# hermosayhl/CNN

Measured on AMD Instinct MI355X. Metric: images/sec (train step, 224x224x3), higher is better.
Workload: dtype f32; 1 GPU; reference AlexNet-style net (cpu/src/alexnet.cpp:10-33: 4x Conv3x3/s2 + ReLU, one MaxPool2x2, Linear 4608->3), full train step (fwd + softmax/CE + bwd + SGD), 224x224x3 fp32, BASELINE configs[1]; per_gpu_batch=256, global_batch=256, parallelism=dp1

## Files before the change

### cnn_amd/csrc/conv_direct.hip

```cpp
#include <cstdlib>

#include "conv_families.h"

using namespace cnn_amd;

namespace {

constexpr int kWaves = 4;
constexpr int kBlock = 64 * kWaves;

template <int CI, int CO, int K, int S>
__global__ __launch_bounds__(kBlock) void conv_direct_fwd(const float* __restrict__ x, const float* __restrict__ w,
                                                          const float* __restrict__ bias, float* __restrict__ y,
                                                          float* __restrict__ y_relu, int B, int H, int W, int Ho,
                                                          int Wo) {
    const int lane = threadIdx.x & 63;
    const int wave = __builtin_amdgcn_readfirstlane(threadIdx.x >> 6);
    const long long rows = (long long)B * Ho;
    for (long long r = (long long)blockIdx.x * kWaves + wave; r < rows; r += (long long)gridDim.x * kWaves) {
        const int b = (int)(r / Ho), p = (int)(r - (long long)b * Ho);
        const float* xb = x + (size_t)b * CI * H * W + (size_t)(p * S) * W;
        float* yb = y + (size_t)b * CO * Ho * Wo + (size_t)p * Wo;
        float* rb = y_relu ? y_relu + (size_t)b * CO * Ho * Wo + (size_t)p * Wo : nullptr;
        for (int q = lane; q < Wo; q += 64) {
// ... 496 lines not shown
    pack_fwd_3_16_3_2_body(w, bias, wp, threadIdx.x, blockDim.x);
}

struct PackJob {
    int kind;
    const float* w;
    const float* bias;
    float* out;
    int CI, CO;
};
struct PackBatch {
    int n;
    PackJob j[8];
};
__global__ void pack_batch(const PackBatch pb) {
    const PackJob& jb = pb.j[blockIdx.y];
    const int tid = blockIdx.x * blockDim.x + threadIdx.x, nt = gridDim.x * blockDim.x;
    if (jb.kind == 0) pack_fwd_3_16_3_2_body(jb.w, jb.bias, jb.out, tid, nt);
    else if (jb.kind == 1) pack_dgrad_3_16_3_2_body(jb.w, jb.out, tid);
    else pack_dgrad_s2_body(jb.w, jb.out, jb.CI, jb.CO, tid, nt);
}

constexpr int kFinThreads = 1024, kFinLanes = 8, kFinN = 16 * 28;
__global__ __launch_bounds__(kFinThreads) void first_layer_finish(const float* __restrict__ slabs, int nslots, float divisor,
                                                                  float* __restrict__ gw, float* __restrict__ gb, float* __restrict__ w,
                                                                  float* __restrict__ bias, float lr, float scale, int scaled,
                                                                  float* __restrict__ fwd_img, float* __restrict__ dgrad_img,
                                                                  float* __restrict__ w_keep, float* __restrict__ bias_keep) {
    __shared__ float red[kFinLanes][kFinN];
    __shared__ float wl[16 * 27], bl[16];
    constexpr int PAIRS = kFinLanes * kFinN, PER = (PAIRS + kFinThreads - 1) / kFinThreads;
    float acc[PER];
    int idx[PER], sl[PER];
#pragma unroll
    for (int q = 0; q < PER; ++q) {
        const int pr = threadIdx.x + q * kFinThreads;
        acc[q] = 0.f;
        sl[q] = pr / kFinN;
        idx[q] = pr - sl[q] * kFinN;
    }
    const bool last_live = threadIdx.x + (PER - 1) * kFinThreads < PAIRS;
    if (!last_live) idx[PER - 1] = 0, sl[PER - 1] = 0;
    constexpr int kBatch = 8;
    for (int s0 = 0; s0 < nslots; s0 += kBatch * kFinLanes) {
        float v[kBatch][PER];
#pragma unroll
        for (int u = 0; u < kBatch; ++u)
#pragma unroll
            for (int q = 0; q < PER; ++q) {
                const int s = s0 + u * kFinLanes + sl[q];
                v[u][q] = slabs[(size_t)(s < nslots ? s : 0) * kFinN + idx[q]];
            }
#pragma unroll
        for (int u = 0; u < kBatch; ++u)
#pragma unroll
            for (int q = 0; q < PER; ++q) {
                const float sum = acc[q] + v[u][q];
                acc[q] = (s0 + u * kFinLanes + sl[q] < nslots) ? sum : acc[q];
            }
    }
#pragma unroll
    for (int q = 0; q < PER; ++q)
        if (q + 1 < PER || last_live) red[sl[q]][idx[q]] = acc[q];
    __syncthreads();
    if (threadIdx.x < kFinN) {
        const int i = threadIdx.x;
        float t = 0.f;
#pragma unroll
        for (int k = 0; k < kFinLanes; ++k) t += red[k][i];
        const float g = t / divisor;
        const int row = i / 28, col = i - row * 28;
        if (col < 27) {
            const int j = row * 27 + col;
            gw[j] = g;
            const float old = w[j];
            if (w_keep) w_keep[j] = old;
            const float v = sgd_one(old, g, lr, scale, scaled != 0);
            w[j] = v;
            wl[j] = v;
        } else {
            if (gb) gb[row] = g;
            const float oldb = bias ? bias[row] : 0.f;
            if (bias && bias_keep) bias_keep[row] = oldb;
            const float v = bias ? sgd_one(oldb, g, lr, scale, scaled != 0) : 0.f;
            if (bias) bias[row] = v;
            bl[row] = v;
        }
    }
    __syncthreads();
    if (fwd_img) pack_fwd_3_16_3_2_body(wl, bl, fwd_img, threadIdx.x, kFinThreads);
    if (dgrad_img) pack_dgrad_3_16_3_2_body(wl, dgrad_img, threadIdx.x);
}

constexpr int kDR = 4;
constexpr int kDSeg = 62;
template <int MODE>
__global__ __launch_bounds__(kBlock) void conv_dgrad_pool_lds_3_16_3_2(const float* __restrict__ dpool, const int32_t* __restrict__ pmask,
                                                                       const float* __restrict__ pooled, const v2f* __restrict__ wp,
                                                                       float* __restrict__ dx, int B, int H, int W, int Ho, int Wo,
                                                                       int ngroups, int nsegs, unsigned m_gs, unsigned m_seg) {
    constexpr bool RM = MODE == 1, PK8 = MODE == 2;
    constexpr int CO = 16, CI = 3, NA = RM ? 3 : 2, ROWS = kDR + 1;
    static_assert(kDR == kWaves, "one block row per wave");
    __shared__ float tile[NA][CO][ROWS][64];
    const int U = (H + 1) / 2, V = (W + 1) / 2, U2 = (U + 1) / 2, V2 = (V + 1) / 2;
    const int PHo = Ho / 2, PWo = Wo / 2, pplane = PHo * PWo, plane = Ho * Wo;
    const int lane = threadIdx.x & 63;
    const int wave = __builtin_amdgcn_readfirstlane(threadIdx.x >> 6);
    const int pbytes = (int)((unsigned)B * CO * pplane * 4u);
    const int pitch8 = pool_mask_pitch(PWo), plane8 = PHo * pitch8;
    const __amdgpu_buffer_rsrc_t rd = __builtin_amdgcn_make_buffer_rsrc((void*)dpool, 0, pbytes, 0x00020000);
    const __amdgpu_buffer_rsrc_t rm = __builtin_amdgcn_make_buffer_rsrc((void*)pmask, 0, PK8 ? (int)((unsigned)B * CO * plane8) : pbytes, 0x00020000);
    const __amdgpu_buffer_rsrc_t rp = __builtin_amdgcn_make_buffer_rsrc((void*)(RM ? pooled : dpool), 0, pbytes, 0x00020000);
    const int item = (int)xcd_swizzle(blockIdx.x, gridDim.x);
    const int gs = ngroups * nsegs;
    const int b = fast_div(item, m_gs, gs);
    const int rem = item - b * gs;
    const int grp = fast_div(rem, m_seg, nsegs), sg = rem - grp * nsegs;
    const int bh0 = grp * kDR, bw0 = sg * kDSeg;
    {
        const int wc = bw0 - 1 + lane;
        const bool cok = wc >= 0 && wc < PWo && lane <= kDSeg;
        constexpr int PER = CO * ROWS / kWaves;
        float vd[PER], vm[PER], vp[RM ? PER : 1];
#pragma unroll
        for (int jj = 0; jj < PER; ++jj) {
            const int j = jj * kWaves + wave;
            const int ch = j / ROWS, r = j - ch * ROWS;
            const int wr = bh0 - 1 + r;
            const unsigned off = (cok && wr >= 0 && wr < PHo) ? (unsigned)(wr * PWo + wc) * 4u : kBufOOB;
            const int so = (b * CO + ch) * pplane * 4;
            vd[jj] = __builtin_bit_cast(float, __builtin_amdgcn_raw_buffer_load_b32(rd, (int)off, so, 0));
            if constexpr (PK8) {
                const unsigned off8 = (off != kBufOOB) ? (unsigned)(wr * pitch8 + wc) : kBufOOB;
                vm[jj] = __builtin_bit_cast(float, (int)__builtin_amdgcn_raw_buffer_load_b8(rm, (int)off8, (b * CO + ch) * plane8, 0));
            } else
                vm[jj] = __builtin_bit_cast(float, __builtin_amdgcn_raw_buffer_load_b32(rm, (int)off, so, 0));
            if constexpr (RM) vp[jj] = __builtin_bit_cast(float, __builtin_amdgcn_raw_buffer_load_b32(rp, (int)off, so, 0));
        }
#pragma unroll
        for (int jj = 0; jj < PER; ++jj) {
            const int j = jj * kWaves + wave;
            const int ch = j / ROWS, r = j - ch * ROWS;
            tile[0][ch][r][lane] = vd[jj];
            tile[1][ch][r][lane] = vm[jj];
            if constexpr (RM) tile[2][ch][r][lane] = vp[jj];
        }
    }
    __syncthreads();
    const int bh = bh0 + wave, bw = bw0 + lane;
    if (bh >= U2) return;
    const bool live = lane < kDSeg && bw < V2;
    const int e00 = (2 * bh - 1) * Wo + (2 * bw - 1);
    v2f acc[4][6];
#pragma unroll
    for (int sb = 0; sb < 4; ++sb)
#pragma unroll
        for (int k = 0; k < 6; ++k) acc[sb][k] = v2f{0.f, 0.f};
    const int l1 = lane < 63 ? lane + 1 : 63;
#pragma unroll 2
    for (int ch = 0; ch < CO; ++ch) {
        float g[4], pl[4];
        int mk[4];
#pragma unroll
        for (int w = 0; w < 4; ++w) {
            const int r = wave + (w >> 1), sl = (w & 1) ? l1 : lane;
            g[w] = tile[0][ch][r][sl];
            mk[w] = __builtin_bit_cast(int, tile[1][ch][r][sl]);
            if constexpr (RM) pl[w] = tile[2][ch][r][sl];
            else pl[w] = 1.f;
        }
        float D[3][3];
        const int cbase = ch * plane + e00;
#pragma unroll
        for (int w = 0; w < 4; ++w) g[w] = (pl[w] <= 0.f) ? 0.f : g[w];
#pragma unroll
        for (int i = 0; i < 3; ++i)
#pragma unroll
            for (int j = 0; j < 3; ++j) {
                const int w = ((i + 1) >> 1) * 2 + ((j + 1) >> 1);
                if constexpr (PK8) D[i][j] = (mk[w] == ((i + 1) & 1) * 2 + ((j + 1) & 1)) ? g[w] : 0.f;
                else D[i][j] = (mk[w] == cbase + i * Wo + j) ? g[w] : 0.f;
            }
        asm volatile("" ::: "memory");
        const v2f* q = wp + ch * 16;
#pragma unroll
        for (int sb = 0; sb < 4; ++sb) {
            const int sr = sb >> 1, sc = sb & 1;
            const v2f a = {D[sr + 1][sc + 1], D[sr + 1][sc + 1]}, bq = {D[sr + 1][sc], D[sr + 1][sc]},
                      c = {D[sr][sc + 1], D[sr][sc + 1]}, e = {D[sr][sc], D[sr][sc]};
            v2f& P0 = acc[sb][0]; v2f& P1 = acc[sb][1]; v2f& P2 = acc[sb][2]; v2f& P3 = acc[sb][3];
            v2f& Q0 = acc[sb][4]; v2f& Q1 = acc[sb][5];
            P0 = __builtin_elementwise_fma(q[0], a, P0);
            P1 = __builtin_elementwise_fma(q[1], a, P1);
            P2 = __builtin_elementwise_fma(q[2], a, P2);
            P3 = __builtin_elementwise_fma(q[3], a, P3);
            Q0 = __builtin_elementwise_fma(q[4], a, Q0);
            Q1 = __builtin_elementwise_fma(q[5], a, Q1);
            P0 = __builtin_elementwise_fma(q[6], bq, P0);
            P2 = __builtin_elementwise_fma(q[7], bq, P2);
            Q0 = __builtin_elementwise_fma(q[8], bq, Q0);
            Q1 = __builtin_elementwise_fma(q[9], bq, Q1);
            P0 = __builtin_elementwise_fma(q[10], c, P0);
            P1 = __builtin_elementwise_fma(q[11], c, P1);
            Q0 = __builtin_elementwise_fma(q[12], c, Q0);
            P0 = __builtin_elementwise_fma(q[13], e, P0);
            Q0 = __builtin_elementwise_fma(q[14], e, Q0);
        }
    }
    if (!live) return;
    float* dxb = dx + (size_t)b * CI * H * W;
    const bool quad = (W & 3) == 0;
#pragma unroll
    for (int ci = 0; ci < CI; ++ci)
#pragma unroll
        for (int rr = 0; rr < 4; ++rr) {
            const int sr = rr >> 1, ph = rr & 1, h = 4 * bh + rr;
            float v[4];
#pragma unroll
            for (int sc = 0; sc < 2; ++sc) {
                const v2f* A = acc[sr * 2 + sc];
                if (ci == 2) {
                    v[2 * sc] = ph ? A[5].x : A[4].x;
                    v[2 * sc + 1] = ph ? A[5].y : A[4].y;
                } else {
                    const v2f lo = ph ? A[2] : A[0], hi = ph ? A[3] : A[1];
                    v[2 * sc] = ci ? lo.y : lo.x;
                    v[2 * sc + 1] = ci ? hi.y : hi.x;
                }
            }
            if (h >= H) continue;
            float* row = dxb + ((size_t)ci * H + h) * W + 4 * (size_t)bw;
            if (quad) {
                {
                    typedef float nt4 __attribute__((ext_vector_type(4)));
                    __builtin_nontemporal_store(nt4{v[0], v[1], v[2], v[3]}, (nt4*)row);
                }
            } else {
#pragma unroll
                for (int k = 0; k < 4; ++k)
                    if (4 * bw + k < W) row[k] = v[k];
            }
        }
}

typedef int v2i __attribute__((ext_vector_type(2)));

template <bool RELU>
__global__ __launch_bounds__(kBlock) void conv_fwd_pk_3_16_3_2(const float* __restrict__ x, const v2f* __restrict__ wp,
                                                               float* __restrict__ y, float* __restrict__ y_relu, int B,
                                                               int H, int W, int Ho, int Wo, int items_per_img,
                                                               unsigned m_ipi, unsigned m_row) {
    constexpr int CI = 3, CO = 16, K = 3;
    const int lane = threadIdx.x & 63;
    const int wave = __builtin_amdgcn_readfirstlane(threadIdx.x >> 6);
    const long long items = (long long)B * items_per_img;
    const int plane = Ho * Wo;
    for (int it = xcd_swizzle(blockIdx.x, gridDim.x) * kWaves + wave; it < (int)items; it += gridDim.x * kWaves) {
        const int b = fast_div(it, m_ipi, items_per_img);
        const int n = (it - b * items_per_img) * 64 + lane;
        const bool live = n < plane;
        const int p = fast_div(live ? n : 0, m_row, Wo), q = (live ? n : 0) - p * Wo;
        const unsigned vo = live ? (unsigned)(2 * p * W + 2 * q) : 0u;
        float patch[CI * K * K];
#pragma unroll
        for (int ci = 0; ci < CI; ++ci)
#pragma unroll
            for (int kx = 0; kx < K; ++kx) {
                const float* rowp = x + (size_t)((b * CI + ci) * H + kx) * W;
                const f3u pr = *(const f3u*)(rowp + vo);
                patch[(ci * K + kx) * K + 0] = pr.x;
                patch[(ci * K + kx) * K + 1] = pr.y;
                patch[(ci * K + kx) * K + 2] = pr.z;
            }
        v2f acc[CO / 2];
#pragma unroll
        for (int j = 0; j < CO / 2; ++j) acc[j] = v2f{0.f, 0.f};
#pragma unroll
        for (int t = 0; t < CI * K * K; ++t) {
            asm volatile("" ::: "memory");
            const v2f* qw = wp + t * (CO / 2);
            const v2f pv = {patch[t], patch[t]};
#pragma unroll
            for (int j = 0; j < CO / 2; ++j) acc[j] = __builtin_elementwise_fma(qw[j], pv, acc[j]);
        }
        if (!live) continue;
        const v2f* qb = wp + CI * K * K * (CO / 2);
        float* yb = y + (size_t)b * CO * plane + n;
        float* rb = RELU ? y_relu + (size_t)b * CO * plane + n : nullptr;
#pragma unroll
        for (int j = 0; j < CO / 2; ++j) {
            const v2f v = acc[j] + qb[j];
            yb[(size_t)(2 * j) * plane] = v.x;
            yb[(size_t)(2 * j + 1) * plane] = v.y;
            if (RELU) {
                rb[(size_t)(2 * j) * plane] = v.x >= 0.f ? v.x : 0.f;
                rb[(size_t)(2 * j + 1) * plane] = v.y >= 0.f ? v.y : 0.f;
            }
        }
    }
}

template <int DBG, bool PK8>
__global__ __launch_bounds__(kBlock) void conv_fwd_pool_pk_3_16_3_2(const float* __restrict__ x, const v2f* __restrict__ wp,
                                                                    float* __restrict__ pooled, int32_t* __restrict__ mask,
                                                                    int B, int H, int W, int Ho, int Wo, int PHo, int PWo,
                                                                    int items_per_img, unsigned m_ipi, unsigned m_prow, int pitch8) {
    constexpr int CI = 3, CO = 16, K = 3;
    const int lane = threadIdx.x & 63;
    const int wave = __builtin_amdgcn_readfirstlane(threadIdx.x >> 6);
    const long long items = (long long)B * items_per_img;
    const int half = 2 * PHo * PWo;
    const int out_bytes = (int)((unsigned)B * CO * PHo * PWo * 4u);
    const int mask_bytes = PK8 ? (int)((unsigned)B * CO * PHo * pitch8) : out_bytes;
    const __amdgpu_buffer_rsrc_t rpool = __builtin_amdgcn_make_buffer_rsrc((void*)pooled, 0, out_bytes, 0x00020000);
    const __amdgpu_buffer_rsrc_t rmask = __builtin_amdgcn_make_buffer_rsrc((void*)(mask ? mask : (int32_t*)pooled), 0, mask ? mask_bytes : out_bytes, 0x00020000);
    for (int it = xcd_swizzle(blockIdx.x, gridDim.x) * kWaves + wave; it < (int)items; it += gridDim.x * kWaves) {
        const int b = fast_div(it, m_ipi, items_per_img);
        const int n2 = (it - b * items_per_img) * 64 + lane;
        const bool live = n2 < half;
        const int pp = (live ? n2 : 0) >> 1, j = n2 & 1;
        const int ph = fast_div(pp, m_prow, PWo), pw = pp - ph * PWo;
        const int q = 2 * pw + j;
        const unsigned vo = live ? (unsigned)(4 * ph * W + 2 * q) : 0u;
        float patch[CI][5][K];
#pragma unroll
        for (int ci = 0; ci < CI; ++ci)
#pragma unroll
            for (int r = 0; r < 5; ++r) {
                const float* rowp = x + (size_t)((b * CI + ci) * H + r) * W;
                const f3u pr = *(const f3u*)(rowp + vo);
                patch[ci][r][0] = pr.x;
                patch[ci][r][1] = pr.y;
                patch[ci][r][2] = pr.z;
            }
        v2f acc0[CO / 2], acc1[CO / 2];
#pragma unroll
        for (int c = 0; c < CO / 2; ++c) acc0[c] = acc1[c] = v2f{0.f, 0.f};
#pragma unroll
        for (int t = 0; t < CI * K * K; ++t) {
            if (DBG != 2 || t == 0) asm volatile("" ::: "memory");
            const int ci = t / 9, kx = (t - ci * 9) / 3, ky = t - ci * 9 - kx * 3;
            const v2f* qw = wp + (DBG == 2 ? 0 : t) * (CO / 2);
            const v2f p0 = {patch[ci][kx][ky], patch[ci][kx][ky]}, p1 = {patch[ci][kx + 2][ky], patch[ci][kx + 2][ky]};
            if (DBG == 1) {
                acc0[t & 7] += p0;
                acc1[t & 7] += p1;
                continue;
            }
#pragma unroll
            for (int c = 0; c < CO / 2; ++c) {
                acc0[c] = __builtin_elementwise_fma(qw[c], p0, acc0[c]);
                acc1[c] = __builtin_elementwise_fma(qw[c], p1, acc1[c]);
            }
        }
        asm volatile("" ::: "memory");
        const v2f* qb = wp + CI * K * K * (CO / 2);
        float bestv[CO];
        int offv[CO];
#pragma unroll
        for (int c = 0; c < CO; ++c) {
            const float bsv = (c & 1) ? qb[c / 2].y : qb[c / 2].x;
            float a = ((c & 1) ? acc0[c / 2].y : acc0[c / 2].x) + bsv;
            float d = ((c & 1) ? acc1[c / 2].y : acc1[c / 2].x) + bsv;
            a = a >= 0.f ? a : 0.f;
            d = d >= 0.f ? d : 0.f;
            const float pa = __builtin_bit_cast(float, __builtin_amdgcn_mov_dpp(__builtin_bit_cast(int, a), 0xB1, 0xf, 0xf, true));
            const float pd = __builtin_bit_cast(float, __builtin_amdgcn_mov_dpp(__builtin_bit_cast(int, d), 0xB1, 0xf, 0xf, true));
            float best = a;
            int off = 0;
            const bool c1 = best < pa;
            best = c1 ? pa : best; off = c1 ? 1 : off;
            const bool c2 = best < d;
            best = c2 ? d : best; off = c2 ? Wo : off;
            const bool c3 = best < pd;
            best = c3 ? pd : best; off = c3 ? Wo + 1 : off;
            bestv[c] = best;
            offv[c] = off;
        }
        const unsigned so_lane = (live && j == 0) ? (unsigned)(ph * PWo + pw) * 4u : kBufOOB;
        const int mbase = 2 * ph * Wo + 2 * pw;
        const int PP4 = PHo * PWo * 4;
        const int soff = b * CO * PP4;
#pragma unroll
        for (int c = 0; c < CO; ++c) __builtin_amdgcn_raw_buffer_store_b32(__builtin_bit_cast(int, bestv[c]), rpool, (int)so_lane, soff + c * PP4, 0);
        if (mask && !PK8) {
#pragma unroll
            for (int c = 0; c < CO; ++c) {
                const int marked = (c * Ho * Wo + mbase + offv[c]) | ((bestv[c] <= 0.f) ? (int)0x80000000 : 0);
                __builtin_amdgcn_raw_buffer_store_b32(marked, rmask, (int)so_lane, soff + c * PP4, 0);
            }
        }
        if (mask && PK8) {
            const unsigned so8 = (live && j == 0) ? (unsigned)(ph * pitch8 + pw) : kBufOOB;
            const int PP1 = PHo * pitch8;
            const int soff8 = b * CO * PP1;
#pragma unroll
            for (int c = 0; c < CO; ++c) {
                const int code = (offv[c] >= Wo ? 2 + (offv[c] - Wo) : offv[c]) | ((bestv[c] <= 0.f) ? 0x80 : 0);
                __builtin_amdgcn_raw_buffer_store_b8((unsigned char)code, rmask, (int)so8, soff8 + c * PP1, 0);
            }
        }
    }
}

__global__ __launch_bounds__(kBlock) void pool_mask_unpack_kernel(const unsigned char* __restrict__ packed, int32_t* __restrict__ mask, long long n,
                                                                  int Co, int Ho, int Wo, int pitch8) {
    const int PHo = Ho / 2, PWo = Wo / 2;
    for (long long i = (long long)blockIdx.x * blockDim.x + threadIdx.x; i < n; i += (long long)gridDim.x * blockDim.x) {
        const int pw = (int)(i % PWo);
        const long long r = i / PWo;
        const int ph = (int)(r % PHo), co = (int)((r / PHo) % Co);
        const int code = packed[r * pitch8 + pw];
        mask[i] = (co * Ho * Wo + (2 * ph + ((code >> 1) & 1)) * Wo + 2 * pw + (code & 1)) | ((code & 0x80) ? (int)0x80000000 : 0);
    }
}

constexpr int kWgX = 7;
template <int kWgDepth, int POOLED>
__global__ __launch_bounds__(kBlock) void conv_wgrad_pk_3_16_3_2(const float* __restrict__ x, const float* __restrict__ dy,
                                                                 const int32_t* __restrict__ pmask, const float* __restrict__ pooled,
                                                                 float* __restrict__ slabs, int B, int H, int W, int Ho,
                                                                 int Wo, int items_per_img, unsigned m_ipi, unsigned m_row) {
    constexpr int CI = 3, CO = 16, NP = 14;
    __shared__ float stage[2][4 * kWgX][64];
    const int lane = threadIdx.x & 63;
    const int wave = __builtin_amdgcn_readfirstlane(threadIdx.x >> 6);
    const long long items = (long long)B * items_per_img;
    const int plane = Ho * Wo;
    const int PHo = Ho / 2, PWo = Wo / 2, pplane = PHo * PWo;
    const int dy_bytes = (int)((unsigned)B * CO * (POOLED ? pplane : plane) * 4u);
    const __amdgpu_buffer_rsrc_t rd = __builtin_amdgcn_make_buffer_rsrc((void*)dy, 0, dy_bytes, 0x00020000);
    const __amdgpu_buffer_rsrc_t rm = __builtin_amdgcn_make_buffer_rsrc((void*)(POOLED ? (const void*)pmask : (const void*)dy), 0, dy_bytes, 0x00020000);
    constexpr bool relu_mask = POOLED == 1;
    const __amdgpu_buffer_rsrc_t rp = __builtin_amdgcn_make_buffer_rsrc((void*)(relu_mask ? pooled : dy), 0, dy_bytes, 0x00020000);
    int row_id[3], row_off[3];
#pragma unroll
    for (int i = 0; i < 3; ++i) {
        const int r = wave * 3 + i < 9 ? wave * 3 + i : 8;
        row_id[i] = r;
        row_off[i] = ((r / 3) * H + (r % 3)) * W;
    }
    if (threadIdx.x < 64) stage[0][27][threadIdx.x] = stage[1][27][threadIdx.x] = 0.f;
    const long long per = (items + gridDim.x - 1) / gridDim.x;
    const long long it_end = (blockIdx.x + 1) * per < items ? (blockIdx.x + 1) * per : items;
    constexpr int ND = POOLED ? 13 : 4;
    f3u lx[kWgDepth][3];
    float ldy[kWgDepth][ND];
    auto issue = [&](long long it, f3u(&ax)[3], float(&ad)[ND]) {
        const bool inr = it < it_end;
        const int iti = inr ? (int)it : 0;
        const int b = fast_div(iti, m_ipi, items_per_img);
        const int n = (iti - b * items_per_img) * 64 + lane;
        const bool live = inr && n < plane;
        const int p = fast_div(live ? n : 0, m_row, Wo), q = (live ? n : 0) - p * Wo;
        const unsigned vx = live ? (unsigned)(2 * p * W + 2 * q) : 0u;
        const float* xb = x + (size_t)b * CI * H * W;
#pragma unroll
        for (int i = 0; i < 3; ++i) ax[i] = *(const f3u*)(xb + row_off[i] + vx);
        if constexpr (POOLED) {
            const bool win = live && (p >> 1) < PHo && (q >> 1) < PWo;
            const unsigned vd = win ? (unsigned)((p >> 1) * PWo + (q >> 1)) * 4u : kBufOOB;
            const int sd = (b * CO + 4 * wave) * pplane * 4;
#pragma unroll
            for (int c = 0; c < 4; ++c) {
                ad[c] = __builtin_bit_cast(float, __builtin_amdgcn_raw_buffer_load_b32(rd, (int)vd, sd + c * pplane * 4, 0));
                ad[4 + c] = __builtin_bit_cast(float, __builtin_amdgcn_raw_buffer_load_b32(rm, (int)vd, sd + c * pplane * 4, 0));
                if constexpr (relu_mask) ad[8 + c] = __builtin_bit_cast(float, __builtin_amdgcn_raw_buffer_load_b32(rp, (int)vd, sd + c * pplane * 4, 0));
                else ad[8 + c] = 1.f;
            }
            ad[12] = __builtin_bit_cast(float, 4 * wave * plane + n);
        } else {
            const unsigned vd = live ? (unsigned)n * 4u : kBufOOB;
            const int sd = (b * CO + 4 * wave) * plane * 4;
#pragma unroll
            for (int c = 0; c < 4; ++c)
                ad[c] = __builtin_bit_cast(float, __builtin_amdgcn_raw_buffer_load_b32(rd, (int)vd, sd + c * plane * 4, 0));
        }
    };

    v2f A[4][NP];
    float bs[4];
#pragma unroll
    for (int c = 0; c < 4; ++c) {
        bs[c] = 0.f;
#pragma unroll
        for (int j = 0; j < NP; ++j) A[c][j] = v2f{0.f, 0.f};
    }
    const long long stride = 1;
    long long it = blockIdx.x * per;
#pragma unroll
    for (int dd = 0; dd < kWgDepth; ++dd) issue(it + dd * stride, lx[dd], ldy[dd]);
    int k = 0;
    auto consume = [&](f3u(&ax)[3], float(&ad)[ND]) {
        float(*st)[64] = stage[k & 1];
#pragma unroll
        for (int i = 0; i < 3; ++i) {
            st[row_id[i] * 3 + 0][lane] = ax[i].x;
            st[row_id[i] * 3 + 1][lane] = ax[i].y;
            st[row_id[i] * 3 + 2][lane] = ax[i].z;
        }
        float d[4];
#pragma unroll
        for (int c = 0; c < 4; ++c) {
            if constexpr (POOLED) {
                const int want = __builtin_bit_cast(int, ad[12]) + c * plane;
                const bool hit = __builtin_bit_cast(int, ad[4 + c]) == want;
                d[c] = (hit && !(ad[8 + c] <= 0.f)) ? ad[c] : 0.f;
            } else {
                d[c] = ad[c];
            }
        }
        __builtin_amdgcn_fence(__ATOMIC_RELEASE, "workgroup", "local");
        __builtin_amdgcn_s_barrier();
        __builtin_amdgcn_fence(__ATOMIC_ACQUIRE, "workgroup", "local");
        issue(it + kWgDepth * stride, ax, ad);
        v2f pv[NP];
#pragma unroll
        for (int j = 0; j < NP; ++j) pv[j] = v2f{st[2 * j][lane], st[2 * j + 1][lane]};
#pragma unroll
        for (int c = 0; c < 4; ++c) {
            const v2f dd = {d[c], d[c]};
            bs[c] += d[c];
#pragma unroll
            for (int j = 0; j < NP; ++j) A[c][j] = __builtin_elementwise_fma(pv[j], dd, A[c][j]);
        }
        ++k;
        it += stride;
    };
    while (it < it_end) {
#pragma unroll
        for (int dd = 0; dd < kWgDepth; ++dd) consume(lx[dd], ldy[dd]);
    }
    float* out = slabs + (size_t)blockIdx.x * CO * 28 + (size_t)(4 * wave) * 28;
#pragma unroll
    for (int c = 0; c < 4; ++c) {
#pragma unroll
        for (int j = 0; j < NP; ++j) {
            float a = A[c][j].x, b2 = A[c][j].y;
#pragma unroll
            for (int o = 32; o >= 1; o >>= 1) {
                a += __shfl_xor(a, o, 64);
                b2 += __shfl_xor(b2, o, 64);
            }
            if (lane == 0) {
                out[c * 28 + 2 * j] = a;
                if (2 * j + 1 < 27) out[c * 28 + 2 * j + 1] = b2;
            }
        }
        float t = bs[c];
#pragma unroll
        for (int o = 32; o >= 1; o >>= 1) t += __shfl_xor(t, o, 64);
        if (lane == 0) out[c * 28 + 27] = t;
    }
}

inline unsigned wave_grid(long long rows) {
    long long need = (rows + kWaves - 1) / kWaves;
    const long long cap = (long long)num_cus() * 32;
    return (unsigned)(need < 1 ? 1 : (need > cap ? cap : need));
}

}

namespace cnn_amd {
bool direct_conv_supported(const cnn_conv2d_desc* d) {
    return d->Ci == 3 && d->Co == 16 && d->k == 3 && d->s == 2 && d->pad == 0 && !CNN_OPT_SET("NO_DIRECT");
}

bool direct_fwd_pk_ok(const cnn_conv2d_desc* d) {
    return (long long)d->B * 3 * d->H * d->W * 4 < (1ll << 31) - 16 && !CNN_OPT_SET("FWD_NOPK");
}
int direct_conv_forward(const cnn_conv2d_desc* d, const float* x, const float* w, const float* bias, float* y,
                        float* y_relu, void* ws, size_t ws_bytes, hipStream_t s, bool prepared) {
    const int Ho = cnn_conv2d_out_dim(d->H, d->k, d->s, 0), Wo = cnn_conv2d_out_dim(d->W, d->k, d->s, 0);
    if ((y_relu != nullptr || prepared) && ws != nullptr && ws_bytes >= 28 * 16 * sizeof(float) && direct_fwd_pk_ok(d)) {
        if (!prepared)
            CNN_KLAUNCH(s, "pack_fwd_weights", (pack_fwd_weights_3_16_3_2<<<1, 256, 0, s>>>(w, bias, (float*)ws)), CONV_TAG(d));
        const int ipi = (Ho * Wo + 63) / 64;
        const long long witems = (long long)d->B * ipi;
        if (y_relu)
            CNN_KLAUNCH(s, "conv_fwd_pk<3,16,3,2>+relu",
                        (conv_fwd_pk_3_16_3_2<true><<<wave_grid(witems), kBlock, 0, s>>>(x, (const v2f*)ws, y, y_relu, d->B, d->H,
                                                                                        d->W, Ho, Wo, ipi, div_magic(ipi), div_magic(Wo))), CONV_TAG(d));
        else
            CNN_KLAUNCH(s, "conv_fwd_pk<3,16,3,2>",
                        (conv_fwd_pk_3_16_3_2<false><<<wave_grid(witems), kBlock, 0, s>>>(x, (const v2f*)ws, y, nullptr, d->B, d->H,
                                                                                         d->W, Ho, Wo, ipi, div_magic(ipi), div_magic(Wo))), CONV_TAG(d));
        return CNN_AMD_OK;
    }
    CNN_REQUIRE(!prepared, "internal: prepared forward without a packed kernel");
    const long long rows = (long long)d->B * Ho;
    CNN_KLAUNCH(s, y_relu ? "conv_direct_fwd<3,16,3,2>+relu" : "conv_direct_fwd<3,16,3,2>",
                (conv_direct_fwd<3, 16, 3, 2><<<wave_grid(rows), kBlock, 0, s>>>(x, w, bias, y, y_relu, d->B, d->H, d->W, Ho, Wo)),
                CONV_TAG(d));
    return CNN_AMD_OK;
}

bool direct_conv_pool_supported(const cnn_conv2d_desc* d) {
    const int Ho = cnn_conv2d_out_dim(d->H, d->k, d->s, 0), Wo = cnn_conv2d_out_dim(d->W, d->k, d->s, 0);
    return direct_conv_supported(d) && direct_fwd_pk_ok(d) && Ho >= 2 && Wo >= 2 && (long long)16 * Ho * Wo < (1ll << 31) &&
           (long long)d->B * 16 * (Ho / 2) * (Wo / 2) * 4 < (1ll << 31) - 16 && !CNN_OPT_SET("NO_POOL_FUSION");
}
bool direct_pool_mask_packed_ok(const cnn_conv2d_desc* d) {
    if (!direct_conv_pool_supported(d) || win_wgrad_slots(d) <= 0 || CNN_OPT_INT("DGRAD_POOL_LDS", 1) == 0) return false;
    if (CNN_OPT_INT("WG_POOL_RD", 0) != 0 || CNN_OPT_INT("POOL_MASK_PACKED", 1) == 0 || !direct_dgrad_pk_ok(d)) return false;
    const int U = (d->H + 1) / 2, V = (d->W + 1) / 2, U2 = (U + 1) / 2, V2 = (V + 1) / 2;
    return (long long)d->B * ((U2 + kDR - 1) / kDR) * ((V2 + kDSeg - 1) / kDSeg) < (1ll << 31);
}
size_t direct_pool_mask_bytes(const cnn_conv2d_desc* d) {
    const int Ho = cnn_conv2d_out_dim(d->H, d->k, d->s, d->pad), Wo = cnn_conv2d_out_dim(d->W, d->k, d->s, d->pad);
    if (Ho < 2 || Wo < 2) return 0;
    if (d->flags & CNN_CONV2D_POOL_MASK_PACKED) return (size_t)d->B * d->Co * (Ho / 2) * pool_mask_pitch(Wo / 2) + 64;
    return (size_t)d->B * d->Co * (Ho / 2) * (Wo / 2) * sizeof(int32_t);
}
int direct_pool_mask_unpack(const cnn_conv2d_desc* d, const void* packed, int32_t* mask, hipStream_t s) {
    const int Ho = cnn_conv2d_out_dim(d->H, d->k, d->s, d->pad), Wo = cnn_conv2d_out_dim(d->W, d->k, d->s, d->pad);
    CNN_REQUIRE(Ho >= 2 && Wo >= 2 && (long long)d->Co * Ho * Wo < (1ll << 31), "cnn_conv2d_pool_mask_unpack: geometry not covered");
    const long long n = (long long)d->B * d->Co * (Ho / 2) * (Wo / 2);
    CNN_KLAUNCH(s, "pool_mask_unpack", (pool_mask_unpack_kernel<<<wave_grid((n + 63) / 64), kBlock, 0, s>>>((const unsigned char*)packed, mask, n, d->Co,
                                                                                                        Ho, Wo, pool_mask_pitch(Wo / 2))), CONV_TAG(d));
    return CNN_AMD_OK;
}
int direct_conv_pool_forward(const cnn_conv2d_desc* d, const float* x, const float* w, const float* bias, float* pooled,
                             int32_t* mask, void* ws, size_t ws_bytes, hipStream_t s, bool prepared) {
    CNN_REQUIRE(direct_conv_pool_supported(d), "cnn_conv2d_relu_maxpool2_forward: geometry not covered (3->16 channels, 3x3 stride 2)");
    CNN_REQUIRE(ws != nullptr && ws_bytes >= 28 * 16 * sizeof(float), "cnn_conv2d_relu_maxpool2_forward: workspace too small");
    const int Ho = cnn_conv2d_out_dim(d->H, d->k, d->s, 0), Wo = cnn_conv2d_out_dim(d->W, d->k, d->s, 0);
    const int PHo = Ho / 2, PWo = Wo / 2;
    if (!prepared)
        CNN_KLAUNCH(s, "pack_fwd_weights", (pack_fwd_weights_3_16_3_2<<<1, 256, 0, s>>>(w, bias, (float*)ws)), CONV_TAG(d));
    const int ipi = (2 * PHo * PWo + 63) / 64;
    const long long witems = (long long)d->B * ipi;
    const int dbg = CNN_MEASURE_INT("DBG", 0);
    const bool pk8 = (d->flags & CNN_CONV2D_POOL_MASK_PACKED) != 0;
    CNN_REQUIRE(!pk8 || direct_pool_mask_packed_ok(d), "cnn_conv2d_relu_maxpool2_forward: packed pool mask not available (cnn_conv2d_pool_mask_packed_supported)");
    const int pitch8 = pool_mask_pitch(PWo);
#define FP_LAUNCH(DBG_, PK8_)                                                                                                  \
    CNN_KLAUNCH(s, PK8_ ? "conv_fwd_pool_pk<3,16,3,2>+m8" : "conv_fwd_pool_pk<3,16,3,2>",                                      \
                (conv_fwd_pool_pk_3_16_3_2<DBG_, PK8_><<<wave_grid(witems), kBlock, 0, s>>>(x, (const v2f*)ws, pooled, mask, d->B, d->H, d->W, Ho, \
                                                                                     Wo, PHo, PWo, ipi, div_magic(ipi), div_magic(PWo), pitch8)),  \
                CONV_TAG(d))
    if (pk8) FP_LAUNCH(0, true);
    else if (dbg == 1) FP_LAUNCH(1, false);
    else if (dbg == 2) FP_LAUNCH(2, false);
    else FP_LAUNCH(0, false);
#undef FP_LAUNCH
    return CNN_AMD_OK;
}

bool direct_dgrad_pk_ok(const cnn_conv2d_desc* d) {
    const int Ho = cnn_conv2d_out_dim(d->H, d->k, d->s, 0), Wo = cnn_conv2d_out_dim(d->W, d->k, d->s, 0);
    return (long long)d->B * 16 * Ho * Wo * 4 < (1ll << 31) - 16 && !CNN_OPT_SET("DG_NOPK");
}
int direct_conv_dgrad(const cnn_conv2d_desc* d, const float* dy, const float* w, float* dx, void* ws, size_t ws_bytes,
                      hipStream_t s, bool prepared) {
    const int Ho = cnn_conv2d_out_dim(d->H, d->k, d->s, 0), Wo = cnn_conv2d_out_dim(d->W, d->k, d->s, 0);
    if (ws != nullptr && ws_bytes >= 16 * 32 * sizeof(float) && direct_dgrad_pk_ok(d)) {
        if (!prepared)
            CNN_KLAUNCH(s, "pack_dgrad_weights", (pack_dgrad_weights_3_16_3_2<<<1, 64, 0, s>>>(w, (float*)ws)), CONV_TAG(d));
        const int V = (d->W + 1) / 2, UVg = ((d->H + 1) / 2) * V;
        const int ipi = (UVg + 63) / 64;
        const long long witems = (long long)d->B * ipi;
        const int dbg = CNN_MEASURE_INT("DBG", 0);
#define PK_LAUNCH(DBG_)                                                                                              \
    CNN_KLAUNCH(s, "conv_dgrad_pk<3,16,3,2>",                                                                       \
                (conv_dgrad_pk_3_16_3_2<4, DBG_><<<wave_grid(witems), kBlock, 0, s>>>(dy, (const v2f*)ws, dx, d->B, d->H, d->W, Ho, \
                                                                                     Wo, ipi, div_magic(ipi), div_magic(V))), \
                CONV_TAG(d))
        if (dbg == 4) PK_LAUNCH(4);
        else if (dbg == 8) PK_LAUNCH(8);
        else if (dbg == 12) PK_LAUNCH(12);
        else PK_LAUNCH(0);
#undef PK_LAUNCH
        return CNN_AMD_OK;
    }
    CNN_REQUIRE(!prepared, "internal: prepared dgrad without a packed kernel");
    const long long rows = (long long)d->B * ((d->H + d->s - 1) / d->s);
    CNN_KLAUNCH(s, "conv_direct_dgrad<3,16,3,2>",
                (conv_direct_dgrad<3, 16, 3, 2, 4><<<wave_grid(rows), kBlock, 0, s>>>(dy, w, dx, d->B, d->H, d->W, Ho, Wo, 0)),
                CONV_TAG(d));
    return CNN_AMD_OK;
}


int direct_conv_dgrad_pooled(const cnn_conv2d_desc* d, const float* dpool, const int32_t* mask, const float* pooled, const float* w,
                             float* dx, void* ws, size_t ws_bytes, hipStream_t s, bool prepared) {
    CNN_REQUIRE(direct_conv_pool_supported(d) && direct_dgrad_pk_ok(d), "cnn_conv2d_backward_data_pooled2: geometry not covered");
    CNN_REQUIRE(ws != nullptr && ws_bytes >= 16 * 32 * sizeof(float), "cnn_conv2d_backward_data_pooled2: workspace too small");
    const int Ho = cnn_conv2d_out_dim(d->H, d->k, d->s, 0), Wo = cnn_conv2d_out_dim(d->W, d->k, d->s, 0);
    if (!prepared)
        CNN_KLAUNCH(s, "pack_dgrad_weights", (pack_dgrad_weights_3_16_3_2<<<1, 64, 0, s>>>(w, (float*)ws)), CONV_TAG(d));
    const int U = (d->H + 1) / 2, V = (d->W + 1) / 2, U2 = (U + 1) / 2, V2 = (V + 1) / 2;
    const int ipi = (U2 * V2 + 63) / 64;
    const long long witems = (long long)d->B * ipi;
    unsigned grid = wave_grid(witems);
    if (const OptVal e = CNN_OPT_VAL("DX0_GRID"))
        if (atoi(e) > 0 && (unsigned)atoi(e) < grid) grid = (unsigned)atoi(e);
    const int ngroups = (U2 + kDR - 1) / kDR, nsegs = (V2 + kDSeg - 1) / kDSeg;
    const long long nitems = (long long)d->B * ngroups * nsegs;
    const bool pk8 = (d->flags & CNN_CONV2D_POOL_MASK_PACKED) != 0;
    CNN_REQUIRE(!pk8 || (direct_pool_mask_packed_ok(d) && pooled == nullptr),
                "cnn_conv2d_backward_data_pooled2: packed pool mask not available here (cnn_conv2d_pool_mask_packed_supported; pooled must be NULL)");
    if (CNN_OPT_INT("DGRAD_POOL_LDS", 1) != 0 && nitems < (1ll << 31)) {
#define DL_LAUNCH(MODE_, NAME_)                                                                                                          \
    CNN_KLAUNCH(s, NAME_,                                                                                                                \
                (conv_dgrad_pool_lds_3_16_3_2<MODE_><<<(unsigned)nitems, kBlock, 0, s>>>(dpool, mask, pooled, (const v2f*)ws, dx, d->B, d->H, d->W, Ho, \
                                                                                         Wo, ngroups, nsegs, div_magic(ngroups * nsegs), div_magic(nsegs))), \
                CONV_TAG(d))
        if (pk8) DL_LAUNCH(2, "conv_dgrad_pk<3,16,3,2>+poolm8");
        else if (pooled) DL_LAUNCH(1, "conv_dgrad_pk<3,16,3,2>+pool");
        else DL_LAUNCH(0, "conv_dgrad_pk<3,16,3,2>+poolm");
#undef DL_LAUNCH
        return CNN_AMD_OK;
    }
    if (pooled)
        CNN_KLAUNCH(s, "conv_dgrad_pk<3,16,3,2>+pool",
                    (conv_dgrad_pool_pk_3_16_3_2<2, true><<<grid, kBlock, 0, s>>>(dpool, mask, pooled, (const v2f*)ws, dx, d->B, d->H,
                                                                                              d->W, Ho, Wo, ipi, div_magic(ipi), div_magic(V2))),
                    CONV_TAG(d));
    else
        CNN_KLAUNCH(s, "conv_dgrad_pk<3,16,3,2>+poolm",
                    (conv_dgrad_pool_pk_3_16_3_2<2, false><<<grid, kBlock, 0, s>>>(dpool, mask, nullptr, (const v2f*)ws, dx, d->B, d->H,
                                                                                               d->W, Ho, Wo, ipi, div_magic(ipi), div_magic(V2))),
                    CONV_TAG(d));
    return CNN_AMD_OK;
}

bool pk_dgrad_s2_supported(const cnn_conv2d_desc* d) {
    const int Ho = cnn_conv2d_out_dim(d->H, d->k, d->s, 0), Wo = cnn_conv2d_out_dim(d->W, d->k, d->s, 0);
    const OptVal e = CNN_OPT_VAL("PK_DGRAD");
    if (e && atoi(e) == 0) return false;
    return d->k == 3 && d->s == 2 && d->pad == 0 && (d->Ci == 16 || (e && d->Ci == 32)) && d->Co % 4 == 0 && d->Co * 9 * d->Ci * 4 <= 144 * 1024 &&
           (long long)d->B * d->Co * Ho * Wo * 4 < (1ll << 31) - 16 && (long long)d->B * (((d->H + 1) / 2) * ((d->W + 1) / 2) + 63) / 64 < (1ll << 30);
}
size_t pk_dgrad_s2_workspace_floats(const cnn_conv2d_desc* d) { return (size_t)d->Co * 9 * d->Ci; }

int pk_dgrad_s2(const cnn_conv2d_desc* d, const float* dy, const float* w, float* dx, void* ws, hipStream_t s, bool prepared,
                const float* relu_below) {
    const int Ho = cnn_conv2d_out_dim(d->H, d->k, d->s, 0), Wo = cnn_conv2d_out_dim(d->W, d->k, d->s, 0);
    const int total = d->Co * 9 * d->Ci;
    if (!prepared)
        CNN_KLAUNCH(s, "pack_dgrad_weights", (pack_dgrad_weights_s2<<<(total + 255) / 256, 256, 0, s>>>(w, (float*)ws, d->Ci, d->Co)),
                    CONV_TAG(d));
    const int V = (d->W + 1) / 2, UVg = ((d->H + 1) / 2) * V;
    const int ipi = (UVg + 63) / 64;
    const long long witems = (long long)d->B * ipi;
    const size_t wl = (size_t)total * sizeof(float);
    if (d->Ci == 16) {
        CNN_KLAUNCH(s, relu_below ? "conv_dgrad_pk_s2<16>+relu" : "conv_dgrad_pk_s2<16>",
                    (conv_dgrad_pk_s2<16, 4, 1><<<wave_grid(witems), kBlock, wl, s>>>(dy, (const v2f*)ws, dx, relu_below, d->B, d->Co, d->H, d->W, Ho,
                                                                                     Wo, ipi, div_magic(ipi), div_magic(V))),
                    CONV_TAG(d));
    } else {
        static DeviceOnce attr_once;
        if (int rc = allow_dynamic_lds(attr_once, 160 * 1024, conv_dgrad_pk_s2<32, 4, 1>)) return rc;
        CNN_KLAUNCH(s, relu_below ? "conv_dgrad_pk_s2<32>+relu" : "conv_dgrad_pk_s2<32>",
                    (conv_dgrad_pk_s2<32, 4, 1><<<wave_grid(witems), kBlock, wl, s>>>(dy, (const v2f*)ws, dx, relu_below, d->B, d->Co, d->H, d->W, Ho,
                                                                                     Wo, ipi, div_magic(ipi), div_magic(V))),
                    CONV_TAG(d));
    }
    return CNN_AMD_OK;
}

int direct_prepare_batch(int n, const ConvPrepJob* jobs, hipStream_t s) {
    PackBatch pb;
    CNN_REQUIRE(n <= (int)(sizeof(pb.j) / sizeof(pb.j[0])), "cnn_conv2d_prepare_filters: %d packed-filter jobs in one call", n);
    pb.n = 0;
    for (int i = 0; i < n; ++i) {
        const cnn_conv2d_desc* d = jobs[i].d;
        if (!direct_conv_supported(d)) pb.j[pb.n++] = PackJob{2, jobs[i].w, nullptr, jobs[i].image, d->Ci, d->Co};
        else if (jobs[i].mode == MODE_FWD) pb.j[pb.n++] = PackJob{0, jobs[i].w, jobs[i].bias, jobs[i].image, 3, 16};
        else pb.j[pb.n++] = PackJob{1, jobs[i].w, nullptr, jobs[i].image, 3, 16};
    }
    if (pb.n > 0) CNN_KLAUNCH(s, "pack_batch", (pack_batch<<<dim3(8, pb.n), 256, 0, s>>>(pb)), "jobs=%d", pb.n);
    return CNN_AMD_OK;
}

int direct_wgrad_slots(const cnn_conv2d_desc* d) {
    if (!direct_conv_supported(d) || CNN_OPT_SET("WG_NOPK")) return 0;
    if (const int ws = win_wgrad_slots(d)) return ws;
    const int Ho = cnn_conv2d_out_dim(d->H, d->k, d->s, 0), Wo = cnn_conv2d_out_dim(d->W, d->k, d->s, 0);
    if ((long long)d->B * 16 * Ho * Wo * 4 >= (1ll << 31) - 16 || (long long)d->B * 3 * d->H * d->W * 4 >= (1ll << 31) - 16) return 0;
    const long long items = (long long)d->B * ((Ho * Wo + 63) / 64);
    const long long cap = (long long)num_cus() * 2;
    return (int)(items < cap ? items : cap);
}

int direct_conv_wgrad(const cnn_conv2d_desc* d, const float* x, const float* dy, float* slabs, hipStream_t s) {
    if (win_wgrad_slots(d) > 0) return win_wgrad_launch(d, x, dy, nullptr, nullptr, slabs, s);
    const int Ho = cnn_conv2d_out_dim(d->H, d->k, d->s, 0), Wo = cnn_conv2d_out_dim(d->W, d->k, d->s, 0);
    const int ipi = (Ho * Wo + 63) / 64;
    CNN_KLAUNCH(s, "conv_wgrad_pk<3,16,3,2>",
                (conv_wgrad_pk_3_16_3_2<3, 0><<<direct_wgrad_slots(d), kBlock, 0, s>>>(x, dy, nullptr, nullptr, slabs, d->B, d->H, d->W,
                                                                                          Ho, Wo, ipi, div_magic(ipi), div_magic(Wo))),
                CONV_TAG(d));
    return CNN_AMD_OK;
}

int direct_conv_wgrad_pooled(const cnn_conv2d_desc* d, const float* x, const float* dpool, const int32_t* mask, const float* pooled,
                             float* slabs, hipStream_t s) {
    CNN_REQUIRE(!(d->flags & CNN_CONV2D_POOL_MASK_PACKED) || (direct_pool_mask_packed_ok(d) && pooled == nullptr),
                "cnn_conv2d_backward_weight_pooled2: packed pool mask not available here (cnn_conv2d_pool_mask_packed_supported; pooled must be NULL)");
    if (win_wgrad_slots(d) > 0) return win_wgrad_launch(d, x, dpool, mask, pooled, slabs, s);
    const int Ho = cnn_conv2d_out_dim(d->H, d->k, d->s, 0), Wo = cnn_conv2d_out_dim(d->W, d->k, d->s, 0);
    const int ipi = (Ho * Wo + 63) / 64;
    if (pooled)
        CNN_KLAUNCH(s, "conv_wgrad_pk<3,16,3,2>+pool",
                    (conv_wgrad_pk_3_16_3_2<3, 1><<<direct_wgrad_slots(d), kBlock, 0, s>>>(x, dpool, mask, pooled, slabs, d->B, d->H, d->W,
                                                                                          Ho, Wo, ipi, div_magic(ipi), div_magic(Wo))),
                    CONV_TAG(d));
    else
        CNN_KLAUNCH(s, "conv_wgrad_pk<3,16,3,2>+poolm",
                    (conv_wgrad_pk_3_16_3_2<3, 2><<<direct_wgrad_slots(d), kBlock, 0, s>>>(x, dpool, mask, nullptr, slabs, d->B, d->H, d->W,
                                                                                          Ho, Wo, ipi, div_magic(ipi), div_magic(Wo))),
                    CONV_TAG(d));
    return CNN_AMD_OK;
}

int direct_first_layer_finish(const cnn_conv2d_desc* d, const float* slabs, int nslots, float divisor, float* gw, float* gb, float* w,
                              float* bias, float lr, float grad_scale, void* fwd_img, void* dgrad_img, float* w_keep, float* bias_keep,
                              hipStream_t s) {
    CNN_REQUIRE(direct_conv_supported(d), "first_layer_finish: geometry not covered");
    CNN_REQUIRE(!fwd_img || direct_fwd_pk_ok(d), "first_layer_finish: this layer has no packed forward kernel");
    CNN_REQUIRE(!dgrad_img || direct_dgrad_pk_ok(d), "first_layer_finish: this layer has no packed data-gradient kernel");
    CNN_KLAUNCH(s, "first_layer_finish",
                (first_layer_finish<<<1, kFinThreads, 0, s>>>(slabs, nslots, divisor, gw, gb, w, bias, lr, grad_scale, grad_scale != 1.0f ? 1 : 0,
                                                              (float*)fwd_img, (float*)dgrad_img, w_keep, bias_keep)),
                CONV_TAG(d));
    return CNN_AMD_OK;
}

}
```

Before: 613,200 images/sec.

## Compute each conv+ReLU+maxpool 2x2 window in one thread by default

Adds a forward path for the first conv layer (3->16, 3x3 stride 2) fused with ReLU and 2x2 max-pool in which each thread computes all four conv outputs of one pooling window. It loads a 3x5x5 input patch once per thread and accumulates 16 channels in chunks of 8 with packed FMA. The old layout used two lanes per pooled output, so each lane re-read overlapping input and the two halves had to be combined. The old path is kept behind FWD_POOL_PAIR. The new path raises register pressure per thread and halves the number of waves launched.

```diff
diff --git a/cnn_amd/csrc/conv_direct.hip b/cnn_amd/csrc/conv_direct.hip
--- a/cnn_amd/csrc/conv_direct.hip
+++ b/cnn_amd/csrc/conv_direct.hip
@@ -822,10 +822,10 @@
 }
 
 template <int DBG, bool PK8>
-__global__ __launch_bounds__(kBlock) void conv_fwd_pool_pk_3_16_3_2(const float* __restrict__ x, const v2f* __restrict__ wp,
-                                                                    float* __restrict__ pooled, int32_t* __restrict__ mask,
-                                                                    int B, int H, int W, int Ho, int Wo, int PHo, int PWo,
-                                                                    int items_per_img, unsigned m_ipi, unsigned m_prow, int pitch8) {
+__device__ __forceinline__ void fwd_pool_pair_body(const float* __restrict__ x, const v2f* __restrict__ wp,
+                                                   float* __restrict__ pooled, int32_t* __restrict__ mask,
+                                                   int B, int H, int W, int Ho, int Wo, int PHo, int PWo,
+                                                   int items_per_img, unsigned m_ipi, unsigned m_prow, int pitch8) {
     constexpr int CI = 3, CO = 16, K = 3;
     const int lane = threadIdx.x & 63;
     const int wave = __builtin_amdgcn_readfirstlane(threadIdx.x >> 6);
@@ -922,6 +922,128 @@
             }
         }
     }
+}
+
+struct __attribute__((packed, aligned(4))) f5u { float a, b, c, d, e; };
+
+template <int DBG, bool PK8>
+__device__ __forceinline__ void fwd_pool_window_body(const float* __restrict__ x, const v2f* __restrict__ wp,
+                                                     float* __restrict__ pooled, int32_t* __restrict__ mask,
+                                                     int B, int H, int W, int Ho, int Wo, int PHo, int PWo,
+                                                     int items_per_img, unsigned m_ipi, unsigned m_prow, int pitch8) {
+    constexpr int CI = 3, CO = 16, K = 3, CP = 4;
+    const int lane = threadIdx.x & 63;
+    const int wave = __builtin_amdgcn_readfirstlane(threadIdx.x >> 6);
+    const long long items = (long long)B * items_per_img;
+    const int PP = PHo * PWo;
+    const int out_bytes = (int)((unsigned)B * CO * PP * 4u);
+    const int mask_bytes = PK8 ? (int)((unsigned)B * CO * PHo * pitch8) : out_bytes;
+    const __amdgpu_buffer_rsrc_t rpool = __builtin_amdgcn_make_buffer_rsrc((void*)pooled, 0, out_bytes, 0x00020000);
+    const __amdgpu_buffer_rsrc_t rmask = __builtin_amdgcn_make_buffer_rsrc((void*)(mask ? mask : (int32_t*)pooled), 0, mask ? mask_bytes : out_bytes, 0x00020000);
+    const int PP4 = PP * 4, PP1 = PHo * pitch8;
+    for (int it = xcd_swizzle(blockIdx.x, gridDim.x) * kWaves + wave; it < (int)items; it += gridDim.x * kWaves) {
+        const int b = fast_div(it, m_ipi, items_per_img);
+        const int n = (it - b * items_per_img) * 64 + lane;
+        const bool live = n < PP;
+        const int ph = fast_div(live ? n : 0, m_prow, PWo), pw = (live ? n : 0) - ph * PWo;
+        const unsigned vo = (unsigned)(4 * ph * W + 4 * pw);
+        v2f pq[CI][5][2], p5[(CI * 5 + 1) / 2];
+        p5[(CI * 5 - 1) / 2] = v2f{0.f, 0.f};
+#pragma unroll
+        for (int ci = 0; ci < CI; ++ci)
+#pragma unroll
+            for (int r = 0; r < 5; ++r) {
+                const float* rowp = x + (size_t)((b * CI + ci) * H + r) * W;
+                const f5u pr = *(const f5u*)(rowp + vo);
+                pq[ci][r][0] = v2f{pr.a, pr.b};
+                pq[ci][r][1] = v2f{pr.c, pr.d};
+                if ((ci * 5 + r) & 1) p5[(ci * 5 + r) / 2].y = pr.e;
+                else p5[(ci * 5 + r) / 2].x = pr.e;
+            }
+        auto px = [&](int ci, int r, int k) -> float {
+            const v2f v = k < 4 ? pq[ci][r][k >> 1] : p5[(ci * 5 + r) / 2];
+            return ((k < 4 ? k : ci * 5 + r) & 1) ? v.y : v.x;
+        };
+        const unsigned so_lane = live ? (unsigned)n * 4u : kBufOOB;
+        const unsigned so8 = live ? (unsigned)(ph * pitch8 + pw) : kBufOOB;
+        const int mbase = 2 * ph * Wo + 2 * pw;
+#pragma unroll
+        for (int h = 0; h < CO / (2 * CP); ++h) {
+            v2f acc[4][CP];
+#pragma unroll
+            for (int ci = 0; ci < CI; ++ci)
+#pragma unroll
+                for (int r = 0; r < 5; ++r) asm("" : "+v"(pq[ci][r][0]), "+v"(pq[ci][r][1]));
+#pragma unroll
+            for (int i = 0; i < (CI * 5 + 1) / 2; ++i) asm("" : "+v"(p5[i]));
+#pragma unroll
+            for (int o = 0; o < 4; ++o)
+#pragma unroll
+                for (int c = 0; c < CP; ++c) acc[o][c] = v2f{0.f, 0.f};
+#pragma unroll
+            for (int t = 0; t < CI * K * K; ++t) {
+                if (DBG != 2 || t == 0) asm volatile("" ::: "memory");
+                const int ci = t / 9, kx = (t - ci * 9) / 3, ky = t - ci * 9 - kx * 3;
+                const v2f* qw = wp + (DBG == 2 ? 0 : t) * (CO / 2) + h * CP;
+#pragma unroll
+                for (int o = 0; o < 4; ++o) {
+                    const float p = px(ci, 2 * (o >> 1) + kx, 2 * (o & 1) + ky);
+                    const v2f pv = {p, p};
+                    if (DBG == 1) {
+                        acc[o][t & (CP - 1)] += pv;
+                        continue;
+                    }
+#pragma unroll
+                    for (int c = 0; c < CP; ++c) acc[o][c] = __builtin_elementwise_fma(qw[c], pv, acc[o][c]);
+                }
+            }
+            asm volatile("" ::: "memory");
+            const v2f* qb = wp + CI * K * K * (CO / 2) + h * CP;
+            float bestv[2 * CP];
+            int offv[2 * CP];
+#pragma unroll
+            for (int c = 0; c < CP; ++c) {
+                const v2f bs = qb[c];
+                const v2f v00 = acc[0][c] + bs, v01 = acc[1][c] + bs, v10 = acc[2][c] + bs, v11 = acc[3][c] + bs;
+#pragma unroll
+                for (int e = 0; e < 2; ++e) {
+                    const float a = e ? v00.y : v00.x, pa = e ? v01.y : v01.x, d = e ? v10.y : v10.x, pd = e ? v11.y : v11.x;
+                    float best = __builtin_fmaxf(a, 0.f);
+                    int off = 0;
+                    const bool c1 = best < pa;
+                    best = c1 ? pa : best; off = c1 ? 1 : off;
+                    const bool c2 = best < d;
+                    best = c2 ? d : best; off = c2 ? (PK8 ? 2 : Wo) : off;
+                    const bool c3 = best < pd;
+                    best = c3 ? pd : best; off = c3 ? (PK8 ? 3 : Wo + 1) : off;
+                    bestv[2 * c + e] = best;
+                    offv[2 * c + e] = best <= 0.f ? (PK8 ? 0x80 : (int)0x80000000) : off;
+                }
+            }
+            const int soff = (b * CO + h * 2 * CP) * PP4;
+#pragma unroll
+            for (int c = 0; c < 2 * CP; ++c) __builtin_amdgcn_raw_buffer_store_b32(__builtin_bit_cast(int, bestv[c]), rpool, (int)so_lane, soff + c * PP4, 0);
+            if (mask && !PK8) {
+#pragma unroll
+                for (int c = 0; c < 2 * CP; ++c)
+                    __builtin_amdgcn_raw_buffer_store_b32((h * 2 * CP + c) * Ho * Wo + mbase + offv[c], rmask, (int)so_lane, soff + c * PP4, 0);
+            }
+            if (mask && PK8) {
+                const int soff8 = (b * CO + h * 2 * CP) * PP1;
+#pragma unroll
+                for (int c = 0; c < 2 * CP; ++c) __builtin_amdgcn_raw_buffer_store_b8((unsigned char)offv[c], rmask, (int)so8, soff8 + c * PP1, 0);
+            }
+        }
+    }
+}
+
+template <int DBG, bool PK8, bool PAIR>
+__global__ __launch_bounds__(kBlock) void conv_fwd_pool_pk_3_16_3_2(const float* __restrict__ x, const v2f* __restrict__ wp,
+                                                                    float* __restrict__ pooled, int32_t* __restrict__ mask,
+                                                                    int B, int H, int W, int Ho, int Wo, int PHo, int PWo,
+                                                                    int items_per_img, unsigned m_ipi, unsigned m_prow, int pitch8) {
+    if (PAIR) fwd_pool_pair_body<DBG, PK8>(x, wp, pooled, mask, B, H, W, Ho, Wo, PHo, PWo, items_per_img, m_ipi, m_prow, pitch8);
+    else fwd_pool_window_body<DBG, PK8>(x, wp, pooled, mask, B, H, W, Ho, Wo, PHo, PWo, items_per_img, m_ipi, m_prow, pitch8);
 }
 
 __global__ __launch_bounds__(kBlock) void pool_mask_unpack_kernel(const unsigned char* __restrict__ packed, int32_t* __restrict__ mask, long long n,
@@ -1150,21 +1272,29 @@
     const int PHo = Ho / 2, PWo = Wo / 2;
     if (!prepared)
         CNN_KLAUNCH(s, "pack_fwd_weights", (pack_fwd_weights_3_16_3_2<<<1, 256, 0, s>>>(w, bias, (float*)ws)), CONV_TAG(d));
-    const int ipi = (2 * PHo * PWo + 63) / 64;
+    const bool pair = CNN_OPT_INT("FWD_POOL_PAIR", 0) != 0;
+    const int ipi = ((pair ? 2 : 1) * PHo * PWo + 63) / 64;
     const long long witems = (long long)d->B * ipi;
     const int dbg = CNN_MEASURE_INT("DBG", 0);
     const bool pk8 = (d->flags & CNN_CONV2D_POOL_MASK_PACKED) != 0;
     CNN_REQUIRE(!pk8 || direct_pool_mask_packed_ok(d), "cnn_conv2d_relu_maxpool2_forward: packed pool mask not available (cnn_conv2d_pool_mask_packed_supported)");
     const int pitch8 = pool_mask_pitch(PWo);
-#define FP_LAUNCH(DBG_, PK8_)                                                                                                  \
+#define FP_LAUNCH(DBG_, PK8_, PAIR_)                                                                                           \
     CNN_KLAUNCH(s, PK8_ ? "conv_fwd_pool_pk<3,16,3,2>+m8" : "conv_fwd_pool_pk<3,16,3,2>",                                      \
-                (conv_fwd_pool_pk_3_16_3_2<DBG_, PK8_><<<wave_grid(witems), kBlock, 0, s>>>(x, (const v2f*)ws, pooled, mask, d->B, d->H, d->W, Ho, \
+                (conv_fwd_pool_pk_3_16_3_2<DBG_, PK8_, PAIR_><<<wave_grid(witems), kBlock, 0, s>>>(x, (const v2f*)ws, pooled, mask, d->B, d->H, d->W, Ho, \
                                                                                      Wo, PHo, PWo, ipi, div_magic(ipi), div_magic(PWo), pitch8)),  \
                 CONV_TAG(d))
-    if (pk8) FP_LAUNCH(0, true);
-    else if (dbg == 1) FP_LAUNCH(1, false);
-    else if (dbg == 2) FP_LAUNCH(2, false);
-    else FP_LAUNCH(0, false);
+    if (pair) {
+        if (pk8) FP_LAUNCH(0, true, true);
+        else if (dbg == 1) FP_LAUNCH(1, false, true);
+        else if (dbg == 2) FP_LAUNCH(2, false, true);
+        else FP_LAUNCH(0, false, true);
+    } else {
+        if (pk8) FP_LAUNCH(0, true, false);
+        else if (dbg == 1) FP_LAUNCH(1, false, false);
+        else if (dbg == 2) FP_LAUNCH(2, false, false);
+        else FP_LAUNCH(0, false, false);
+    }
 #undef FP_LAUNCH
     return CNN_AMD_OK;
 }
```

Measured after the change: 648,800 images/sec, median of 6. 1.06x the previous value.
